# alessandroragano/nomad

Hardware: AMD Instinct MI355X
Metric: clips/sec embedded + NxM NOMAD distances, 16kHz x 4s batches (higher is better)
Workload: dtype f32; 1 GPU; configs[1]: batch=256 x 64000 samples (T=199) per GPU, wav2vec2-base + projection head fp32, 224 deg x 32*N ref float64 distances + means; deg_per_gpu=224, ref_total=32, parallelism=clip-sharded x1, all-gather of ref embeddings, collective=none (single process, no process group)

## Files before the change

### nomad_amd/build.py

```python
from __future__ import annotations

import os
import shutil
import subprocess
import time

HERE = os.path.dirname(os.path.abspath(__file__))
CSRC = os.path.join(HERE, "csrc")
LIB = os.path.join(HERE, "libnomad_hip.so")
DIAG_LIB = os.path.join(HERE, "libnomad_diag.so")
SOURCES = ["nomad_hip.hip", "nomad_gemm_f32.hip", "nomad_gemm_bf16.hip"]
HEADERS = sorted(f for f in os.listdir(CSRC) if f.endswith(".h")) + [os.path.join("..", "..", "include", "nomad_hip.h")]


def hipcc_path() -> str:
    for cand in (os.environ.get("HIPCC"), shutil.which("hipcc"), "/opt/rocm/bin/hipcc"):
        if cand and os.path.exists(cand):
            return cand
    raise RuntimeError("hipcc not found; the HIP libraries cannot be built")


def needs_build(lib: str = LIB) -> bool:
    if not os.path.exists(lib):
        return True
    t = os.path.getmtime(lib)
    deps = [os.path.join(CSRC, s) for s in SOURCES + HEADERS] + [os.path.abspath(__file__)]
    return any(os.path.getmtime(d) > t for d in deps if os.path.exists(d))


NO_PACKED_FP32 = ["-Xclang", "-target-feature", "-Xclang", "-packed-fp32-ops"]


def pk_path(lib: str) -> str:
    return lib[:-3] + "_pk.so"


VARIANTS = {"gelu1": ["-DNOMAD_GELU_BF16_FORM=1"],
            "gelu2": ["-DNOMAD_GELU_BF16_FORM=2"],
            "poswino1": ["-DNOMAD_POSCONV_WINO_LEVELS=1"],
            "gelu_tail6": ["-DNOMAD_GELU_F32_FORM=2"]}


def variant_path(lib: str, name: str) -> str:
    return lib[:-3] + f"_{name}.so"


def _flags(lib: str, diag: bool, verbose: bool):
    flags = ["--offload-arch=gfx950", "-O3", "-std=c++17", "-fPIC", "-Wall", "-Wno-unused-function", "-pthread"]
    for name, defs in VARIANTS.items():
        if lib.endswith(f"_{name}.so"):
            flags = defs + flags
    if os.environ.get("NOMAD_PACKED_FP32", "0") != "1" and not lib.endswith("_pk.so"):
        flags = NO_PACKED_FP32 + flags
    else:
        flags.insert(0, "-DNOMAD_PACKED_FP32_BUILD=1")
    if diag:
        flags.insert(0, "-DNOMAD_DIAG")
    if verbose:
        flags.insert(0, "-Rpass-analysis=kernel-resource-usage")
    return flags


class _Job:

    def __init__(self, lib: str, diag: bool, verbose: bool = False):
        self.lib, self.t0 = lib, time.perf_counter()
        self.tmp = lib + f".tmp{os.getpid()}"
        self.flags = _flags(lib, diag, verbose)
        self.objs = [f"{lib}.{os.path.splitext(s)[0]}.{os.getpid()}.o" for s in SOURCES]
        self.procs = [subprocess.Popen([hipcc_path(), *self.flags, "-c", os.path.join(CSRC, s), "-o", o],
                                       stdout=subprocess.PIPE, stderr=subprocess.PIPE, text=True) for s, o in zip(SOURCES, self.objs)]

    def _cleanup(self):
        for f in self.objs + [self.tmp]:
            if os.path.exists(f):
                os.remove(f)

    def finish(self) -> float:
        errs = []
        for p in self.procs:
            out, err = p.communicate()
            if p.returncode != 0:
                errs.append(out + err)
        if errs:
            self._cleanup()
            raise RuntimeError("hipcc failed:\n" + "\n".join(errs))
        link = subprocess.run([hipcc_path(), "--offload-arch=gfx950", "-shared", "-fPIC", "-pthread", "-o", self.tmp, *self.objs],
                              capture_output=True, text=True)
        if link.returncode != 0:
            self._cleanup()
            raise RuntimeError("hipcc (link) failed:\n" + link.stdout + link.stderr)
        os.replace(self.tmp, self.lib)
        self._cleanup()
# ... 37 lines not shown
```

### nomad_amd/csrc/conv_s2_f32.hip.h

```cpp
#pragma once
#include "gemm_f32.hip.h"

namespace nomad {

struct ConvS2Params {
    const float* X;
    const float* W;
    float* Y;
    float* Upre;
    int pairs;
    int tiles_m;
    int L, Lin, ppc;
    unsigned ppc_magic;
    int ppc_shift;
    const int* pp;
    const int* opref;
    const int* ipref;
    int nclips;
};

struct ConvS2Cfg {
    static constexpr int BMP = 128, BN = 128, NT = 512;
    static constexpr int STAGE = 8 * 1024 + 132;
    static constexpr int ZOFF = 8 * 1024;
    static constexpr int LDS_BYTES = 2 * STAGE * 4;
};

struct PairRows {
    long long in0, in_last, out0;
    bool odd_ok;
};

template <bool RAGGED>
__device__ __forceinline__ PairRows conv_s2_pair(const ConvS2Params& p, int s) {
    PairRows r;
    if (RAGGED) {
        int lo = 0, hi = p.nclips;
        while (hi - lo > 1) {
            const int mid = (lo + hi) >> 1;
            if (p.pp[mid] <= s) lo = mid;
            else hi = mid;
        }
        const int j = s - p.pp[lo];
        const int L = p.opref[lo + 1] - p.opref[lo];
        r.in0 = (long long)p.ipref[lo] + 4 * j;
        r.in_last = (long long)p.ipref[lo + 1] - 1;
        r.out0 = (long long)p.opref[lo] + 2 * j;
        r.odd_ok = 2 * j + 1 < L;
    } else {
        const int c = p.ppc_magic ? fast_div(s, p.ppc_magic, p.ppc_shift) : (p.ppc == 1 ? s : 0);
        const int j = s - c * p.ppc;
        r.in0 = (long long)c * p.Lin + 4 * j;
        r.in_last = (long long)c * p.Lin + p.Lin - 1;
        r.out0 = (long long)c * p.L + 2 * j;
        r.odd_ok = 2 * j + 1 < p.L;
    }
    return r;
}

template <bool RAGGED>
__global__ __launch_bounds__(512, 4) void conv_s2_f32_kernel(const ConvS2Params p) {
    using Cfg = ConvS2Cfg;
    extern __shared__ __attribute__((aligned(16))) float smem[];
    const int tid = threadIdx.x, lane = tid & 63;
    const int wave = __builtin_amdgcn_readfirstlane(tid >> 6);
    const int wm = wave >> 1, wn = wave & 1;
    const int nwg = p.tiles_m * 4;
    const int wg = xcd_remap(blockIdx.x, nwg);
    const int tile_m = wg >> 2, tile_n = wg & 3;
    const int m0 = tile_m * Cfg::BMP, n0 = tile_n * Cfg::BN;

    if (tid < 2 * 33) *reinterpret_cast<f32x4*>(smem + (tid / 33) * Cfg::STAGE + Cfg::ZOFF + (tid % 33) * 4) = (f32x4){0.f, 0.f, 0.f, 0.f};

    const long long tile_in0 = conv_s2_pair<RAGGED>(p, m0).in0;
    const float* const a_tile = uniform_ptr(p.X + tile_in0 * 512);
    const float* const b_tile = uniform_ptr(p.W + (long long)n0 * 1536);
    int v1a, v1b;
    {
        const int r1 = tid >> 2, lc = (tid & 3) ^ ((r1 >> 2) & 3);
        const int s = min(m0 + r1, p.pairs - 1);
        const PairRows pr = conv_s2_pair<RAGGED>(p, s);
        v1a = (int)(((pr.in0 + 2 - tile_in0) * 512 + lc * 4) * 4);
        v1b = (r1 * 1536 + lc * 4) * 4;
    }
    const int f0 = wave >> 2;
    int v2a[3], v2b;
    {
        const int r = (tid & 255) >> 1, lc = (tid & 1) ^ ((r >> 3) & 1);
        const int s = min(m0 + r, p.pairs - 1);
        const PairRows pr = conv_s2_pair<RAGGED>(p, s);
#pragma unroll
        for (int i = 0; i < 3; ++i) {
            const int f = i == 2 ? 4 : f0 + 2 * i;
            const long long row = min(pr.in0 + f, pr.in_last);
            v2a[i] = (int)(((row - tile_in0) * 512 + lc * 4) * 4);
        }
        v2b = (r * 1536 + lc * 4) * 4;
    }
    auto issue = [&](const int q, const int buf) {
        float* st = smem + buf * Cfg::STAGE + wave * 256;
        if (q < 32) {
            const int k0 = q * 16;
            dma16_buffer(a_tile, (lptr_t)(st), v1a, k0 * 4);
            dma16_buffer(b_tile, (lptr_t)(st + 2048), v1b, k0 * 4);
            dma16_buffer(b_tile, (lptr_t)(st + 4096), v1b, (k0 + 1024) * 4);
        } else {
            const int k0 = (q - 32) * 8;
            dma16_buffer(a_tile, (lptr_t)(st), v2a[0], k0 * 4);
            dma16_buffer(a_tile, (lptr_t)(st + 2048), v2a[1], k0 * 4);
            if (f0 == 0) dma16_buffer(a_tile, (lptr_t)(st + 4096), v2a[2], k0 * 4);
            else dma16_buffer(b_tile, (lptr_t)(st + 4096), v2b, k0 * 4);
            dma16_buffer(b_tile, (lptr_t)(st + 6144), v2b, ((1 + f0) * 512 + k0) * 4);
        }
    };

    const int fi = lane & 15, g = lane >> 4;
    const int ra = wm * 32 + fi, rb = wn * 64 + fi;
    const int sw1 = (g ^ ((fi >> 2) & 3)) * 4;
    const int o1a = ra * 16 + sw1, o1b = 2048 + rb * 16 + sw1;
    const int sw2 = ((g & 1) ^ (fi >> 3)) * 4;
    const bool lo = g < 2;
    const int oEF = (lo ? 0 : 1024) + ra * 8 + sw2;
    const int oES = lo ? 2048 + ra * 8 + sw2 : Cfg::ZOFF;
    const int oOF = (lo ? 3072 : 4096) + ra * 8 + sw2;
    const int oOS = lo ? Cfg::ZOFF : 2048 + ra * 8 + sw2;
    const int oBE = (lo ? 5120 : 6144) + rb * 8 + sw2;
    const int oBO = (lo ? 6144 : 7168) + rb * 8 + sw2;

    f32x4 E[2][4], O[2][4];
#pragma unroll
    for (int si = 0; si < 2; ++si)
#pragma unroll
        for (int sj = 0; sj < 4; ++sj) E[si][sj] = (f32x4){0.f, 0.f, 0.f, 0.f};

    auto rd = [&](const float* base, int off) { return *reinterpret_cast<const f32x4*>(base + off); };
    auto mm = [&](f32x4 (&acc)[2][4], const f32x4 (&a)[2], const f32x4 (&b)[4]) {
#pragma unroll
        for (int c = 0; c < 4; ++c)
#pragma unroll
            for (int si = 0; si < 2; ++si)
#pragma unroll
                for (int sj = 0; sj < 4; ++sj) acc[si][sj] = __builtin_amdgcn_mfma_f32_16x16x4f32(b[sj][c], a[si][c], acc[si][sj], 0, 0, 0);
    };
    auto step1 = [&](const float* st) {
        f32x4 a[2], b[4];
#pragma unroll
        for (int si = 0; si < 2; ++si) a[si] = rd(st, o1a + si * 256);
#pragma unroll
        for (int sj = 0; sj < 4; ++sj) {
            const f32x4 u = rd(st, o1b + sj * 256), v = rd(st, o1b + 2048 + sj * 256);
#pragma unroll
            for (int e = 0; e < 4; ++e) b[sj][e] = u[e] + v[e];
        }
        mm(E, a, b);
    };
    auto operand = [&](const float* st, int of, int os, f32x4 (&a)[2]) {
#pragma unroll
        for (int si = 0; si < 2; ++si) {
            const f32x4 u = rd(st, of + si * 128), v = rd(st, os + si * 128);
#pragma unroll
            for (int e = 0; e < 4; ++e) a[si][e] = u[e] - v[e];
        }
    };
    auto step2 = [&](const float* st) {
        f32x4 a[2], b[4];
        operand(st, oEF, oES, a);
#pragma unroll
        for (int sj = 0; sj < 4; ++sj) b[sj] = rd(st, oBE + sj * 128);
        mm(E, a, b);
        asm volatile("" ::: "memory");
        __builtin_amdgcn_sched_barrier(0);
        operand(st, oOF, oOS, a);
#pragma unroll
        for (int sj = 0; sj < 4; ++sj) b[sj] = rd(st, oBO + sj * 128);
        mm(O, a, b);
    };

    auto wait_step = [] {
        asm volatile("s_waitcnt vmcnt(0)" ::: "memory");
        __syncthreads();
    };
    float* const st0 = smem;
    float* const st1 = smem + Cfg::STAGE;
    issue(0, 0);
    for (int q = 0; q < 32; q += 2) {
        wait_step();
        issue(q + 1, 1);
        step1(st0);
        wait_step();
        issue(q + 2, 0);
        step1(st1);
    }
#pragma unroll
    for (int si = 0; si < 2; ++si)
#pragma unroll
        for (int sj = 0; sj < 4; ++sj) O[si][sj] = E[si][sj];
    for (int q = 32; q < 96; q += 2) {
        wait_step();
        issue(q + 1, 1);
        step2(st0);
        wait_step();
        if (q + 2 < 96) issue(q + 2, 0);
        step2(st1);
    }

    int lane_e = lane;
    asm volatile("" : "+v"(lane_e));
    const int col = n0 + wn * 64 + 4 * (lane_e >> 4);
#pragma unroll
    for (int si = 0; si < 2; ++si) {
        const int s = m0 + wm * 32 + (lane_e & 15) + 16 * si;
        if (s >= p.pairs) continue;
        const PairRows pr = conv_s2_pair<RAGGED>(p, s);
        const long long ie = pr.out0 * 512 + col, io = ie + 512;
#pragma unroll
        for (int sj = 0; sj < 4; ++sj) {
            f32x4 ve = E[si][sj], vo = O[si][sj];
            if (p.Upre) {
                *reinterpret_cast<f32x4*>(p.Upre + ie + sj * 16) = ve;
                if (pr.odd_ok) *reinterpret_cast<f32x4*>(p.Upre + io + sj * 16) = vo;
            }
#pragma unroll
            for (int e = 0; e < 4; ++e) {
                ve[e] = gelu_erf(ve[e]);
                vo[e] = gelu_erf(vo[e]);
            }
            *reinterpret_cast<f32x4*>(p.Y + ie + sj * 16) = ve;
            if (pr.odd_ok) *reinterpret_cast<f32x4*>(p.Y + io + sj * 16) = vo;
        }
    }
}

}
```

### nomad_amd/csrc/nomad_ctx.hip.h

```cpp
#pragma once
#include <hip/hip_runtime.h>

#include <algorithm>
#include <cmath>
#include <cstdarg>
#include <cstdio>
#include <cstdlib>
#include <cstring>
#include <atomic>
#include <mutex>
#include <string>
#include <vector>

#include "../../include/nomad_hip.h"

#include "dtypes.hip.h"
#include "gemm_f32.hip.h"

#define NOMAD_INTERNAL __attribute__((visibility("hidden")))

using namespace nomad;

inline thread_local char g_err[512] = "";

// ... 20 lines not shown
constexpr long long kPairScratchDoubles = 1 << 21;
constexpr int kCdistMaxD = 4096;
constexpr int kEventChunk = 8192;
const int* const kNoInts = nullptr;
const hipStream_t kNoStream = reinterpret_cast<hipStream_t>(~uintptr_t(0));

}

struct LayerDev {
    float *qkv_w, *qkv_b, *o_w, *o_b, *ln1_w, *ln1_b, *fc1_w, *fc1_b, *fc2_w, *fc2_b, *ln2_w, *ln2_b;
};


struct Tuning {
    bool splitk_lnb_fuse = true;
    bool splitk_ln_fuse = true;
    bool f32_conv_wino = true;
    bool f32_posconv_wino = true;
    int bf16_attn_tail = 0;
    int bf16_ln_rows = 4;
    int p9_short = 1;
    bool attn_bwd_small = true;
    bool p9_wl = false;
    bool p9_late = true;
    int p9_skew = 0;
    int concurrent_parts = 1;
};

#ifdef NOMAD_DIAG
static void tuning_from_env(Tuning& t) {
    auto geti = [](const char* n, int d) { const char* e = getenv(n); return e ? atoi(e) : d; };
    auto getb = [](const char* n, bool d) { const char* e = getenv(n); return e ? atoi(e) != 0 : d; };
    t.splitk_ln_fuse = getb("NOMAD_SPLITK_LN", t.splitk_ln_fuse);
    t.splitk_lnb_fuse = getb("NOMAD_SPLITK_LNB", t.splitk_lnb_fuse);
    t.f32_conv_wino = getb("NOMAD_F32_CONV_WINO", t.f32_conv_wino);
    t.f32_posconv_wino = getb("NOMAD_F32_POSCONV_WINO", t.f32_posconv_wino);
    t.bf16_attn_tail = geti("NOMAD_BF16_ATTN_TAIL", t.bf16_attn_tail);
    t.bf16_ln_rows = geti("NOMAD_BF16_LN_ROWS", t.bf16_ln_rows);
    t.p9_short = geti("NOMAD_BF16_P9_SHORT", t.p9_short);
    t.p9_skew = geti("NOMAD_BF16_P9_SKEW", t.p9_skew);
    t.p9_late = getb("NOMAD_BF16_P9_LATE", t.p9_late);
    t.p9_wl = getb("NOMAD_BF16_P9_WL", t.p9_wl);
    t.attn_bwd_small = getb("NOMAD_ATTN_BWD_SMALL", t.attn_bwd_small);
}
#endif

struct nomad_ctx {
    int device = 0;
    int num_cus = 256;
    Tuning tune;
    bool keep = false;
    float* conv0_w = nullptr;
    float* conv_w[7] = {};
    float *gn_w = nullptr, *gn_b = nullptr, *fln_w = nullptr, *fln_b = nullptr;
    float *proj_w = nullptr, *proj_b = nullptr;
    float *pos_w = nullptr, *pos_b = nullptr;
    float* pos_wt = nullptr;
    float *eln_w = nullptr, *eln_b = nullptr;
    LayerDev layers[NOMAD_NUM_LAYERS] = {};
    float *emb_w = nullptr, *emb_b = nullptr;
    float* splitk_part = nullptr;
    float* splitk_cur = nullptr;
    size_t splitk_cur_floats = 0;
    bool splitk_ok = false;
    struct PendingLn {
        const float* gamma = nullptr;
        const float* beta = nullptr;
        float* out = nullptr;
        float* out2 = nullptr;
        bool armed = false, done = false;
    } pending_ln;
    struct PendingLnBwd {
        const float* x = nullptr;
        const float* g2 = nullptr;
        const float* gamma = nullptr;
        float* out = nullptr;
        bool armed = false, done = false;
    } pending_lnb;
    std::vector<std::pair<hipStream_t, double*>> pair_scratch;
    std::mutex pair_mu;
    bool bwd_ready = false;
    float* conv_bw_even[7] = {};
    float* conv_bw_odd[7] = {};
    float* conv_bw2[7] = {};
    float* proj_wT = nullptr;
    float* pos_wb = nullptr;
    float *qkv_wT[NOMAD_NUM_LAYERS] = {}, *o_wT[NOMAD_NUM_LAYERS] = {}, *fc1_wT[NOMAD_NUM_LAYERS] = {},
          *fc2_wT[NOMAD_NUM_LAYERS] = {};
    bool bf16_ready = false;
    bf16_t* conv_w16[7] = {};
    bf16_t* conv0_wfrag = nullptr;
    bf16_t *proj_w16 = nullptr, *pos_w16 = nullptr;
    bf16_t* pos_wfrag16 = nullptr;
    bf16_t *qkv_w16[NOMAD_NUM_LAYERS] = {}, *o_w16[NOMAD_NUM_LAYERS] = {}, *fc1_w16[NOMAD_NUM_LAYERS] = {},
           *fc2_w16[NOMAD_NUM_LAYERS] = {};
    float* qkv_b16[NOMAD_NUM_LAYERS] = {};
    bool x3_ready = false;
    bf16s_t* conv_wx[7] = {};
    bf16s_t* proj_wx = nullptr;
    bf16s_t* pos_wx = nullptr;
    float* pos_bx = nullptr;
    bf16s_t *qkv_wx[NOMAD_NUM_LAYERS] = {}, *o_wx[NOMAD_NUM_LAYERS] = {}, *fc1_wx[NOMAD_NUM_LAYERS] = {},
            *fc2_wx[NOMAD_NUM_LAYERS] = {};
    bool train_ready = false;
    float *theta = nullptr, *grad = nullptr, *adam_m = nullptr, *adam_v = nullptr;
    double *pos_nrm2 = nullptr, *tap_partial = nullptr, *tap_dot = nullptr;
// ... 53 lines not shown
        c->p_fl[cls] += flops;
        c->p_n[cls] += 1;
        if (cls2 >= 0) {
            c->p_fl[cls2] += flops;
            c->p_n[cls2] += 1;
        }
        slot = c->ev_used;
        c->ev_class[slot / 2] = cls | ((cls2 + 1) << 8);
        c->ev_used += 2;
        (void)hipEventRecord(c->ev[slot], s);
    }
    ~Scope() {
        if (slot >= 0) (void)hipEventRecord(c->ev[slot + 1], s);
    }
};

RowMap plain_map(int M, int ld) { return RowMap{0, 0, M > 0 ? M : 1, ld}; }

int occ_pad(int occ, int lds) {
    if (occ <= 0) return 0;
    const int budget = (160 * 1024 / occ) & ~255;
    return budget > lds ? budget - lds : 0;
}

GemmParams dense(const float* A, int lda, const float* W, const float* bias, const float* R, float* C, int M, int N,
                 int K, int gelu) {
    GemmParams p{};
    p.A = A;
    p.amap = plain_map(M, lda);
    p.kchunk = K;
    p.kstride = 0;
    p.W = W;
    p.ldw = K;
    p.C = C;
    p.cmap = plain_map(M, N);
    p.bias = bias;
    p.R = R;
    p.rmap = plain_map(M, N);
    p.M = M;
    p.N = N;
    p.K = K;
    p.n_valid = N;
    p.gelu = gelu;
    return p;
}

}

NOMAD_INTERNAL int run_gemm(nomad_ctx* c, GemmParams p, int groups, int tile, hipStream_t s, int occ = 0);
NOMAD_INTERNAL int gemm_f32_dispatch(nomad_ctx* c, GemmParams p, int groups, int tile, hipStream_t s, int occ);
NOMAD_INTERNAL hipError_t gemm_f32_n48_split(const GemmParams& q, int groups, hipStream_t s, int S);
NOMAD_INTERNAL int pick_tile(const nomad_ctx* c, int M, int N, int K);
NOMAD_INTERNAL int mixed_split_rows(const nomad_ctx* c, int M, int N);
NOMAD_INTERNAL int run_conv_s2_f32(nomad_ctx* c, const float* X, const float* W, float* Y, float* Upre, int B, int Lin, int L,
                                   const int* pp, const int* opref, const int* ipref, int pairs, hipStream_t s);
NOMAD_INTERNAL int run_gemm_bf16(nomad_ctx* c, GemmParams p, int groups, hipStream_t s, int tile = -1);
#ifdef NOMAD_DIAG
NOMAD_INTERNAL int gemm_f32_timeline_read(unsigned long long* out_host, int n);
NOMAD_INTERNAL int gemm_bf16_timeline_read(unsigned long long* out_host, int n);
#endif
```

### nomad_amd/csrc/nomad_gemm_f32.hip

```cpp
#include "nomad_ctx.hip.h"
#include "conv_s2_f32.hip.h"

int gemm_f32_dispatch(nomad_ctx* c, GemmParams p, int groups, int tile, hipStream_t s, int occ) {
    if (tile == 29 && occ == 0) occ = 4;
    const double flops = 2.0 * p.M * (double)p.n_valid * p.K * groups;
    Scope sc(c, s, NOMAD_K_GEMM, flops, tile == 33 ? NOMAD_K_GEMM_BIG : ((tile == 34 || tile == 31 || tile == 48) ? NOMAD_K_GEMM_FINE : -1));
    hipError_t e;
    if (c->gemm_x3 && tile == 48 && p.N == 64)
        tile = 37;
    if (c->gemm_x3 && (tile == 31 || tile == 34 || tile == 37) && p.N % 128 == 0 &&
        (long long)((p.M + 127) / 128) * (p.N / 128) >= 512)
        tile = 20;
    const bool plain_cr = p.c_colblk == 0 && p.cmap.clip_rows >= p.M && !p.cmap.pref &&
                          (!p.R || (p.rmap.clip_rows >= p.M && !p.rmap.pref)) && (!p.DG || (p.dgmap.clip_rows >= p.M && !p.dgmap.pref));
    if (c->gemm_x3 && plain_cr && (tile == 20 || tile == 31 || tile == 34 || tile == 37)) {
        constexpr int T = 16 | 32;
        switch (tile) {
            case 20: e = launch_gemm_glds<128, 128, 32, 2, 2, 2, false, 12 | T, true>(p, groups, s, occ_pad(occ, GldsCfg<128, 128, 32, 2, 2>::LDS_BYTES)); break;
            case 31: e = launch_gemm_glds<128, 128, 32, 4, 2, 2, false, 12 | T, true>(p, groups, s, occ_pad(occ, GldsCfg<128, 128, 32, 4, 2>::LDS_BYTES)); break;
            case 34: e = launch_gemm_glds<128, 64, 32, 4, 2, 3, false, 12 | T, true>(p, groups, s); break;
            default: e = launch_gemm_glds<64, 64, 32, 2, 2, 3, false, 12 | T, true>(p, groups, s); break;
        }
        if (e != hipSuccess) return fail(NOMAD_ERR_HIP, "gemm (bf16x3 products) launch: %s", hipGetErrorString(e));
        return 0;
// ... 212 lines not shown
        Scope sc(c, st, NOMAD_K_GEMM, 2.0 * M * (double)N * K, NOMAD_K_GEMM_BIG);
        constexpr int V = 13 | 16 | 64 | 16384;
        if (R) HIP_TRY((launch_gemm_mixed<V | 32768, V | 32768>(pp, m1, st)));
        else HIP_TRY((launch_gemm_mixed<V | 1024, V | 1024>(pp, m1, st)));
        return 0;
    }
    if (tile == 97 || tile == 98) {
        if (N % 128 || K % 32 || gelu || !R) return fail(NOMAD_ERR_INVALID, "nomad_diag_gemm: tile %d needs N %% 128 == 0, K %% 32 == 0, a residual and no GELU", tile);
        GemmParams pp = dense(A, K, W, bias, R, C, M, N, K, gelu);
        hipStream_t st = static_cast<hipStream_t>(stream);
        Scope sc(c, st, NOMAD_K_GEMM, 2.0 * M * (double)N * K, NOMAD_K_GEMM_BIG);
        if (tile == 97) HIP_TRY((launch_gemm_glds<256, 128, 16, 4, 2, 3, false, 13 | 16 | 64 | 16384 | 32768>(pp, 1, st)));
        else HIP_TRY((launch_gemm_glds<128, 128, 32, 4, 2, 2, false, 12 | 16 | 16384 | 32768>(pp, 1, st, occ_pad(0, GldsCfg<128, 128, 32, 4, 2>::LDS_BYTES))));
        return 0;
    }
    if (tile >= 88 && tile <= 93) {
        if (N % 128 || K % 32) return fail(NOMAD_ERR_INVALID, "nomad_diag_gemm: N %% 128 or K %% 32 != 0");
        GemmParams pp = dense(A, K, W, bias, R, C, M, N, K, gelu);
        hipStream_t st = static_cast<hipStream_t>(stream);
        Scope sc(c, st, NOMAD_K_GEMM, 2.0 * M * (double)N * K, NOMAD_K_GEMM_BIG);
        constexpr int L = 16384;
        switch (tile) {
            case 88: HIP_TRY((launch_gemm_glds<256, 128, 16, 4, 2, 3, false, 13 | 16 | L>(pp, 1, st))); break;
            case 89: HIP_TRY((launch_gemm_glds<256, 128, 16, 4, 2, 3, false, 13 | 16 | 1024 | L>(pp, 1, st))); break;
            case 90: HIP_TRY((launch_gemm_glds<256, 128, 16, 4, 2, 3, false, 13 | 16 | 64 | 1024 | L>(pp, 1, st))); break;
            case 91: HIP_TRY((launch_gemm_glds<256, 128, 16, 4, 2, 3, false, 13 | 16 | 64 | L>(pp, 1, st))); break;
            case 92: HIP_TRY((launch_gemm_glds<128, 128, 32, 4, 2, 2, false, 12 | 16 | L>(pp, 1, st, occ_pad(0, GldsCfg<128, 128, 32, 4, 2>::LDS_BYTES)))); break;
            default: HIP_TRY((launch_gemm_glds<128, 128, 32, 4, 2, 2, false, 12 | 16 | 1024 | L>(pp, 1, st, occ_pad(0, GldsCfg<128, 128, 32, 4, 2>::LDS_BYTES)))); break;
        }
        return 0;
    }
    if (tile == 84 || tile == 85) {
        if (N % 128 || K % 16) return fail(NOMAD_ERR_INVALID, "nomad_diag_gemm: N %% 128 or K %% 16 != 0");
        GemmParams pp = dense(A, K, W, bias, R, C, M, N, K, gelu);
        Scope sc(c, static_cast<hipStream_t>(stream), NOMAD_K_GEMM, 2.0 * M * (double)N * K, NOMAD_K_GEMM_BIG);
        if (tile == 85) return fail(NOMAD_ERR_INVALID, "nomad_diag_gemm: tile 85 (BK = 8) went with the 16x16x4 products (16-deep k groups)");
        HIP_TRY((launch_gemm_glds<256, 128, 16, 4, 2, 3, false, 13 | 16 | 64 | 1024>(pp, 1, static_cast<hipStream_t>(stream))));
        return 0;
    }
#else
    if (tile == 84 || tile == 85 || (tile >= 88 && tile <= 95) || (tile >= 97 && tile <= 99))
        return fail(NOMAD_ERR_INVALID, "gemm tile id %d is not in this library (experimental instantiations live in libnomad_diag.so)", tile);
#endif
    if (tile < 0 || (tile > 47 && (tile < 60 || tile > 81) && tile != 86)) return fail(NOMAD_ERR_INVALID, "nomad_diag_gemm: tile id %d", tile);
    const int bn = (tile == 46 || tile == 47) ? 64 : tile >= 60 ? (tile == 67 ? 256 : 128) : kBN[tile], bk = tile == 46 ? 32 : tile == 47 ? 16 : tile >= 60 ? (tile == 73 ? 32 : 16) : kBK[tile];
    if (N % bn || K % bk) return fail(NOMAD_ERR_INVALID, "nomad_diag_gemm: N %% %d or K %% %d != 0", bn, bk);
    GemmParams p = dense(A, K, W, bias, R, C, M, N, K, gelu);
    p.group_m = group_m;
    return run_gemm(c, p, 1, tile, static_cast<hipStream_t>(stream), occ);
}

}

int run_conv_s2_f32(nomad_ctx* c, const float* X, const float* W, float* Y, float* Upre, int B, int Lin, int L, const int* pp,
                    const int* opref, const int* ipref, int pairs, hipStream_t s) {
    ConvS2Params p{};
    p.X = X;
    p.W = W;
    p.Y = Y;
    p.Upre = Upre;
    p.pairs = pairs;
    p.tiles_m = (pairs + ConvS2Cfg::BMP - 1) / ConvS2Cfg::BMP;
    p.nclips = B;
    if (ipref) {
        p.pp = pp;
        p.opref = opref;
        p.ipref = ipref;
    } else {
        p.L = L;
        p.Lin = Lin;
        p.ppc = (L + 1) / 2;
        if (Lin < 2 * L + 1 || pairs != B * p.ppc) return fail(NOMAD_ERR_INVALID, "conv_s2: %d clips of %d -> %d frames, %d pairs", B, Lin, L, pairs);
        p.ppc_magic = 0;
        p.ppc_shift = 0;
        if (B > 1 && p.ppc > 1) fast_div_magic((unsigned)p.ppc, &p.ppc_magic, &p.ppc_shift);
    }
    const double flops = 2.0 * (double)pairs * 512 * 2560;
    Scope sc(c, s, NOMAD_K_GEMM, flops, NOMAD_K_GEMM_BIG);
    static LdsAttrOnce attr_u, attr_r;
    hipError_t e;
    if (ipref) {
        if ((e = attr_r.ensure(reinterpret_cast<const void*>(conv_s2_f32_kernel<true>), ConvS2Cfg::LDS_BYTES)) != hipSuccess)
            return fail(NOMAD_ERR_HIP, "conv_s2 attribute: %s", hipGetErrorString(e));
        hipLaunchKernelGGL(conv_s2_f32_kernel<true>, dim3(p.tiles_m * 4), dim3(ConvS2Cfg::NT), ConvS2Cfg::LDS_BYTES, s, p);
    } else {
        if ((e = attr_u.ensure(reinterpret_cast<const void*>(conv_s2_f32_kernel<false>), ConvS2Cfg::LDS_BYTES)) != hipSuccess)
            return fail(NOMAD_ERR_HIP, "conv_s2 attribute: %s", hipGetErrorString(e));
        hipLaunchKernelGGL(conv_s2_f32_kernel<false>, dim3(p.tiles_m * 4), dim3(ConvS2Cfg::NT), ConvS2Cfg::LDS_BYTES, s, p);
    }
    if ((e = hipGetLastError()) != hipSuccess) return fail(NOMAD_ERR_HIP, "conv_s2 launch: %s", hipGetErrorString(e));
    return 0;
}

#ifdef NOMAD_DIAG
extern "C" {
int nomad_diag_conv_s2(nomad_ctx* c, const float* X, const float* W, float* Y, float* U, int B, const int* lin_host, int ragged,
                       void* stream) {
    if (!c || !X || !W || !Y || !lin_host || B <= 0) return fail(NOMAD_ERR_INVALID, "nomad_diag_conv_s2: bad argument");
    std::vector<int> meta(3 * (size_t)(B + 1), 0);
    for (int b = 0; b < B; ++b) {
        const int lin = lin_host[b], L = lin >= 3 ? (lin - 3) / 2 + 1 : 0;
        if (L <= 0 || (!ragged && lin != lin_host[0])) return fail(NOMAD_ERR_INVALID, "nomad_diag_conv_s2: clip %d of %d frames", b, lin);
        meta[b + 1] = meta[b] + (L + 1) / 2;
        meta[(B + 1) + b + 1] = meta[(B + 1) + b] + L;
        meta[2 * (B + 1) + b + 1] = meta[2 * (B + 1) + b] + lin;
    }
    hipStream_t s = static_cast<hipStream_t>(stream);
    int* d = nullptr;
    HIP_TRY(hipMalloc(&d, sizeof(int) * meta.size()));
    int rc = 0;
    if (hipMemcpy(d, meta.data(), sizeof(int) * meta.size(), hipMemcpyHostToDevice) != hipSuccess) rc = fail(NOMAD_ERR_HIP, "nomad_diag_conv_s2: copy");
    const int lin0 = lin_host[0], L0 = (lin0 - 3) / 2 + 1;
    if (rc == 0)
        rc = ragged ? run_conv_s2_f32(c, X, W, Y, U, B, 0, 0, d, d + (B + 1), d + 2 * (B + 1), meta[B], s)
                    : run_conv_s2_f32(c, X, W, Y, U, B, lin0, L0, nullptr, nullptr, nullptr, meta[B], s);
    if (rc == 0 && hipStreamSynchronize(s) != hipSuccess) rc = fail(NOMAD_ERR_HIP, "nomad_diag_conv_s2: kernel");
    (void)hipFree(d);
    return rc;
}
}
#endif
```

### nomad_amd/csrc/nomad_hip.hip

```cpp
#include "nomad_ctx.hip.h"

#include "attention.hip.h"
#include "attention_bf16_v3.hip.h"
#include "posconv_bf16_slab.hip.h"
#include "attention_f32_v2.hip.h"
#include "attention_bwd.hip.h"
#include "backward.hip.h"
#include "frontend.hip.h"
#include "gemm_bf16.hip.h"
#include "gemm_bf16_8phase.hip.h"
#include "gemm_bf16_p9.hip.h"
#include "gemm_bf16x3.hip.h"
#include "gemm_f32.hip.h"
#ifdef NOMAD_DIAG
#endif
#include "pairwise.hip.h"
#include "posconv_wino_f32.hip.h"
#include "rowops.hip.h"
#include "train.hip.h"
#include "wav_reader.h"

namespace {

struct Shapes {
// ... 763 lines not shown
            if ((long long)m.size() < info[i].frames) m.resize((size_t)info[i].frames);
            status[i] = wav::read_one(paths[i], info[i], m.data(), raw[(size_t)t]);
            if (status[i] != NOMAD_OK) return;
            if (kern_rate[(size_t)t] != info[i].sample_rate) {
                kern[(size_t)t] = wav::make_resample_kernel(info[i].sample_rate, target_rate);
                kern_rate[(size_t)t] = info[i].sample_rate;
            }
            wav::resample_into(m.data(), info[i].frames, kern[(size_t)t], dst,
                               wav::resampled_frames(info[i].frames, info[i].sample_rate, target_rate));
        });
    } catch (const std::exception& e) {
        return fail(NOMAD_ERR_IO, "nomad_wav_read_rows: %s", e.what());
    }
    for (int i = 0; i < n; ++i)
        if (status[i] != NOMAD_OK) return fail(status[i], "nomad_wav_read_rows: %s: %s", paths[i], status[i] == NOMAD_ERR_IO ? "read failed" : "unsupported encoding");
    return NOMAD_OK;
}

int nomad_num_frames(int n_samples) {
    Shapes s;
    return make_shapes(1, n_samples, &s) ? s.T : 0;
}

int nomad_create(nomad_ctx** out, int device, const nomad_weights* w) {
    if (!out || !w) return fail(NOMAD_ERR_INVALID, "nomad_create: null argument");
    int ndev = 0;
    if (hipGetDeviceCount(&ndev) != hipSuccess || ndev <= 0 || device < 0 || device >= ndev)
        return fail(NOMAD_ERR_NO_DEVICE, "nomad_create: no HIP device %d (count %d); this engine has no CPU path",
                    device, ndev);
    hipDeviceProp_t prop;
    HIP_TRY(hipGetDeviceProperties(&prop, device));
    if (strncmp(prop.gcnArchName, "gfx950", 6) != 0)
        return fail(NOMAD_ERR_NO_DEVICE, "nomad_create: device %d is %s, kernels are built for gfx950 only", device,
                    prop.gcnArchName);
    HIP_TRY(hipSetDevice(device));
    nomad_ctx* c = new nomad_ctx();
    c->device = device;
    c->num_cus = prop.multiProcessorCount > 0 ? prop.multiProcessorCount : 256;
#ifdef NOMAD_DIAG
    tuning_from_env(c->tune);
#endif
    int rc = 0;
    auto up = [&](const float* h, size_t n, float** d) {
        if (rc == 0) rc = upload(c, h, n, d);
    };
    up(w->conv_w[0], 512 * 10, &c->conv0_w);
    for (int i = 1; i < 7 && rc == 0; ++i) {
        const int k = kConvK[i];
        std::vector<float> r((size_t)512 * k * 512);
        for (int n = 0; n < 512; ++n)
            for (int ci = 0; ci < 512; ++ci)
                for (int t = 0; t < k; ++t) r[(size_t)n * k * 512 + t * 512 + ci] = w->conv_w[i][((size_t)n * 512 + ci) * k + t];
        up(r.data(), r.size(), &c->conv_w[i]);
    }
    up(w->gn_w, 512, &c->gn_w);
    up(w->gn_b, 512, &c->gn_b);
    up(w->feat_ln_w, 512, &c->fln_w);
    up(w->feat_ln_b, 512, &c->fln_b);
    up(w->proj_w, 768 * 512, &c->proj_w);
    up(w->proj_b, 768, &c->proj_b);
    if (rc == 0) {
        std::vector<double> nrm(128, 0.0);
        for (size_t o = 0; o < 768; ++o)
            for (size_t ci = 0; ci < 48; ++ci)
                for (size_t t = 0; t < 128; ++t) {
                    const double v = w->pos_v[(o * 48 + ci) * 128 + t];
                    nrm[t] += v * v;
                }
        std::vector<float> sc(128);
        for (int t = 0; t < 128; ++t) sc[t] = (float)((double)w->pos_g[t] / std::sqrt(nrm[t]));
        std::vector<float> r((size_t)16 * 64 * 6144, 0.f);
        for (size_t g = 0; g < 16; ++g)
            for (size_t n = 0; n < 48; ++n)
                for (size_t ci = 0; ci < 48; ++ci)
                    for (size_t t = 0; t < 128; ++t)
                        r[(g * 64 + n) * 6144 + t * 48 + ci] = w->pos_v[((g * 48 + n) * 48 + ci) * 128 + t] * sc[t];
        up(r.data(), r.size(), &c->pos_w);
        if (rc == 0 && c->tune.f32_posconv_wino) {
            void* d = nullptr;
            const hipError_t e = hipMalloc(&d, sizeof(float) * 16 * kPwOps * 64 * kPwK);
            if (e != hipSuccess) rc = fail(NOMAD_ERR_HIP, "nomad_create: pos-conv weights: %s", hipGetErrorString(e));
            else {
                c->allocs.push_back(d);
                c->pos_wt = static_cast<float*>(d);
                rc = rebuild_posconv_wino_weights(c, nullptr);
                if (rc == 0 && hipStreamSynchronize(nullptr) != hipSuccess) rc = fail(NOMAD_ERR_HIP, "nomad_create: pos-conv weights: kernel");
            }
        }
    }
    up(w->pos_b, 768, &c->pos_b);
    up(w->enc_ln_w, 768, &c->eln_w);
    up(w->enc_ln_b, 768, &c->eln_b);
    for (int l = 0; l < NOMAD_NUM_LAYERS && rc == 0; ++l) {
        const nomad_layer_weights& lw = w->layers[l];
        LayerDev& d = c->layers[l];
        std::vector<float> qkv((size_t)2304 * 768), qb(2304);
        for (size_t i = 0; i < (size_t)768 * 768; ++i) {
            qkv[i] = lw.q_w[i] * 0.125f;
            qkv[(size_t)768 * 768 + i] = lw.k_w[i];
            qkv[(size_t)2 * 768 * 768 + i] = lw.v_w[i];
        }
        for (int i = 0; i < 768; ++i) {
            qb[i] = lw.q_b[i] * 0.125f;
            qb[768 + i] = lw.k_b[i];
            qb[1536 + i] = lw.v_b[i];
        }
// ... 84 lines not shown
    float *pwq = nullptr, *pws = nullptr;
    int* pwmeta = nullptr;
};

static int forward_run(nomad_ctx* c, const float* wav, const BatchGeom& g, const F32Bufs& bf, const float* head_w,
                       const float* head_b, float* emb, float* layers_out, float* splitk_block, size_t splitk_floats, hipStream_t s,
                       const Saved* sv, bool features = false) {
    if (g.ragged() && splitk_block) return fail(NOMAD_ERR_INVALID, "fp32 forward: split-K needs an equal-length batch");
    const int B = g.B, T = g.T, M = (int)g.rows[6];
    const int depth = c->encoder_depth;
    if (depth < NOMAD_NUM_LAYERS && (!layers_out || features)) return refuse_cut(c, "fp32 forward");
    float* const loss_block = (sv == nullptr && layers_out != nullptr && splitk_block != nullptr) ? splitk_block : nullptr;
    const SplitKScope splitk(c, (sv != nullptr || loss_block != nullptr) && !c->train_ready && !g.ragged());
    float* const prev_cur = c->splitk_cur;
    const size_t prev_cur_floats = c->splitk_cur_floats;
    c->splitk_cur = sv != nullptr ? c->splitk_part : loss_block;
    c->splitk_cur_floats = sv != nullptr ? kSplitKPartFloats : loss_block != nullptr ? splitk_floats : 0;
    struct CurRestore {
        nomad_ctx* c;
        float* v;
        size_t n;
        ~CurRestore() { c->splitk_cur = v; c->splitk_cur_floats = n; }
    } cur_restore{c, prev_cur, prev_cur_floats};
    int rc;
    const bool reg = sv != nullptr;
    const DropCfg d_in = make_drop(c, reg ? c->p_input : 0.f), d_res = make_drop(c, reg ? c->p_drop : 0.f),
                  d_att = make_drop(c, reg ? c->p_attn : 0.f);
    int nbr = 1;
    unsigned bmask[4] = {reg ? c->layer_mask : 0xFFFu, 0xFFFu, 0xFFFu, 0xFFFu};
    if (reg && c->branches > 1) {
        if (B % c->branches) return fail(NOMAD_ERR_INVALID, "nomad_embed_train: B=%d is not %d equal branches", B, c->branches);
        nbr = c->branches;
        for (int i = 0; i < nbr; ++i) bmask[i] = c->branch_mask[i];
    }
    const long long act = (long long)M * 768;

    float* gn_scale = sv ? sv->gn_scale : bf.scale;
    float* gn_shift = sv ? sv->gn_shift : bf.shift;
    {
        Scope sc(c, s, NOMAD_K_FRONT, 0.0);
        launch_wav_stats(wav, g.wav_ld, g.L[0], g.max_l0, B, bf.stats, g.lens, s);
        hipLaunchKernelGGL(gn_fold_kernel, dim3(B), dim3(512), 0, s, bf.stats, c->conv0_w, c->gn_w, c->gn_b, g.L[0],
                           gn_scale, gn_shift, sv ? sv->gn_mean : nullptr, sv ? sv->gn_rstd : nullptr, g.lens);
    }
    {
        Scope sc(c, s, NOMAD_K_FRONT, 2.0 * (double)g.rows[0] * 512 * 10);
        hipLaunchKernelGGL(conv0_gn_gelu_kernel<float>, dim3((g.max_l0 + kConv0Frames - 1) / kConv0Frames, B), dim3(256), 0, s,
                           wav, g.wav_ld, g.L[0], c->conv0_w, gn_scale, gn_shift, bf.conv[0], g.lens, g.pref[0]);
    }
    HIP_TRY(hipGetLastError());

    for (int i = 1; i < 7; ++i) {
        if (conv_wino(c, i)) {
            if ((rc = run_conv_s2_f32(c, bf.conv[i - 1], c->conv_w[i], bf.conv[i], sv ? sv->u[i] : nullptr, B, g.L[i - 1], g.L[i],
                                      g.pairpref[i], g.pref[i], g.pref[i - 1], (int)g.pairs[i], s)))
                return rc;
            continue;
        }
        GemmParams p{};
        p.A = bf.conv[i - 1];
        p.amap = g.conv_amap[i];
        p.K = kConvK[i] * 512;
        p.kchunk = p.K;
        p.W = c->conv_w[i];
        p.ldw = p.K;
        p.C = (sv && i == 6) ? sv->c6 : bf.conv[i];
        p.Upre = sv ? sv->u[i] : nullptr;
        p.M = (int)g.rows[i];
        p.N = 512;
        p.n_valid = 512;
        p.cmap = plain_map(p.M, 512);
        p.rmap = p.cmap;
        p.gelu = 1;
        if ((rc = run_gemm(c, p, 1, pick_tile(c, p.M, 512, p.K), s))) return rc;
    }

    if ((rc = run_layernorm(c, sv ? sv->c6 : bf.conv[6], c->fln_w, c->fln_b, bf.featln, nullptr, M, 512, s)))
        return rc;
    float* xpad = bf.xpad;
    {
        Scope sc(c, s, NOMAD_K_ROW, 0.0);
        hipLaunchKernelGGL(zero_pad_rows_kernel<float>, dim3(16 * B), dim3(256), 0, s, xpad, T, g.pref[6], g.ppref, B);
    }
    {
        GemmParams p = dense(bf.featln, 512, c->proj_w, c->proj_b, nullptr, xpad, M, 768, 512, 0);
        p.cmap = g.pad_map;
        p.c_colblk = 48;
        p.c_colblk_stride = g.grp_stride;
        if ((rc = run_gemm(c, p, 1, pick_tile(c, M, 768, 512), s))) return rc;
    }
    if (d_in.threshold) {
        Scope sc(c, s, NOMAD_K_ROW, 0.0);
        hipLaunchKernelGGL(dropout_groups_kernel, dim3(M), dim3(192), 0, s, xpad, T, g.grp_stride, d_in, kSiteInput, g.pref[6], g.ppref, B);
    }
    if (posconv_wino(c)) {
        if (!bf.pwq || !bf.pws) return fail(NOMAD_ERR_INVALID, "fp32 forward: no workspace for the pos-conv operands");
        if ((rc = run_posconv_wino(c, xpad, c->pos_wt, c->pos_b, sv ? sv->y0 : bf.y, sv ? sv->upc : nullptr, g.pos_wino, bf.pwq, bf.pws, bf.pwmeta, s)))
            return rc;
    } else {
        GemmParams p{};
        p.A = xpad;
        p.amap = g.pos_amap;
        p.a_goff = g.grp_stride;
        p.K = 6144;
        p.kchunk = 6144;
        p.W = c->pos_w;
        p.ldw = 6144;
        p.w_goff = 64LL * 6144;
// ... 1707 lines not shown
            v.push_back({b + "self_attn.out_proj.bias", q.o_b, 768});
            v.push_back({b + "self_attn_layer_norm.weight", q.ln1_w, 768});
            v.push_back({b + "self_attn_layer_norm.bias", q.ln1_b, 768});
            v.push_back({b + "fc1.weight", q.fc1_w, (size_t)3072 * 768});
            v.push_back({b + "fc1.bias", q.fc1_b, 3072});
            v.push_back({b + "fc2.weight", q.fc2_w, (size_t)768 * 3072});
            v.push_back({b + "fc2.bias", q.fc2_b, 768});
            v.push_back({b + "final_layer_norm.weight", q.ln2_w, 768});
            v.push_back({b + "final_layer_norm.bias", q.ln2_b, 768});
        }
        const std::string fe = p + "feature_extractor.conv_layers.";
        v.push_back({fe + "0.0.weight", o.conv0_w, 512 * 10});
        v.push_back({fe + "0.2.weight", o.gn_w, 512});
        v.push_back({fe + "0.2.bias", o.gn_b, 512});
        for (int i = 1; i < 7; ++i) v.push_back({fe + std::to_string(i) + ".0.weight", o.conv_w[i], (size_t)512 * 512 * kConvK[i]});
        v.push_back({"embedding_layer.1.weight", o.emb_w, 256 * 768});
        v.push_back({"embedding_layer.1.bias", o.emb_b, 256});
        return v;
    }();
    return segs;
}

void rebuild_conv_bwd_weights(nomad_ctx* c, hipStream_t s) {
    auto transpose = [&](const float* in, int ld_in, float* out, int ld_out, int R, int C) {
        hipLaunchKernelGGL(transpose_kernel, dim3((C + 31) / 32, (R + 31) / 32), dim3(32, 8), 0, s, in, ld_in, out, ld_out, R, C);
    };
    for (int i = 1; i <= 4; ++i) {
        transpose(c->conv_w[i] + 2 * 512, 1536, c->conv_bw_even[i], 1024, 512, 512);
        transpose(c->conv_w[i], 1536, c->conv_bw_even[i] + 512, 1024, 512, 512);
        transpose(c->conv_w[i] + 512, 1536, c->conv_bw_odd[i], 512, 512, 512);
    }
    for (int i = 5; i <= 6; ++i)
        transpose(c->conv_w[i], 1024, c->conv_bw2[i], 512, 512, 1024);
}

int refresh_weights(nomad_ctx* c, hipStream_t s) {
    const ParamOffsets po = make_param_offsets();
    auto transpose = [&](const float* in, int ld_in, float* out, int ld_out, int R, int C) {
        hipLaunchKernelGGL(transpose_kernel, dim3((C + 31) / 32, (R + 31) / 32), dim3(32, 8), 0, s, in, ld_in, out, ld_out, R, C);
    };
    hipLaunchKernelGGL(tap_dot_partial_kernel, dim3(576), dim3(256), 0, s, c->theta + po.pos_v, (const float*)nullptr,
                       c->tap_partial);
    hipLaunchKernelGGL(tap_sum_final_kernel, dim3(1), dim3(1024), 0, s, c->tap_partial, 576, c->pos_nrm2);
    hipLaunchKernelGGL(posconv_fold_kernel, dim3(768), dim3(256), 0, s, c->theta + po.pos_v, c->theta + po.pos_g,
                       c->pos_nrm2, c->pos_w);
    hipLaunchKernelGGL(posconv_bwd_weight_kernel, dim3(16 * 64), dim3(256), 0, s, c->pos_w, c->pos_wb);
    if (c->pos_wt)
        if (int rc = rebuild_posconv_wino_weights(c, s)) return rc;
    transpose(c->proj_w, 512, c->proj_wT, 768, 768, 512);
    for (int i = 1; i < 7; ++i) {
        const long long n = 512LL * 512 * kConvK[i];
        hipLaunchKernelGGL(conv_repack_kernel, dim3((unsigned)((n + 255) / 256)), dim3(256), 0, s, c->theta + po.conv_w[i], c->conv_w[i],
                           kConvK[i]);
    }
    rebuild_conv_bwd_weights(c, s);
    for (int l = 0; l < NOMAD_NUM_LAYERS; ++l) {
        const LayerDev& d = c->layers[l];
        const LayerOffsets& lo = po.L[l];
        const long long w4 = (long long)2304 * 768 / 4, q4 = (long long)768 * 768 / 4;
        hipLaunchKernelGGL(scale_rows_kernel, dim3((unsigned)((w4 + 255) / 256)), dim3(256), 0, s,
                           reinterpret_cast<const float4*>(c->theta + lo.qkv_w), reinterpret_cast<float4*>(d.qkv_w), w4, q4, 0.125f);
        hipLaunchKernelGGL(scale_rows_kernel, dim3(3), dim3(256), 0, s, reinterpret_cast<const float4*>(c->theta + lo.qkv_b),
                           reinterpret_cast<float4*>(d.qkv_b), 576LL, 192LL, 0.125f);
        transpose(d.qkv_w, 768, c->qkv_wT[l], 2304, 2304, 768);
        transpose(d.o_w, 768, c->o_wT[l], 768, 768, 768);
        transpose(d.fc1_w, 768, c->fc1_wT[l], 3072, 3072, 768);
        transpose(d.fc2_w, 3072, c->fc2_wT[l], 768, 768, 3072);
    }
    HIP_TRY(hipGetLastError());
    c->bf16_ready = false;
    c->x3_ready = false;
    return 0;
}

}

extern "C" {

int nomad_set_gemm_precision(nomad_ctx* c, int mode) {
    if (!c || (mode != 0 && mode != 1)) return fail(NOMAD_ERR_INVALID, "nomad_set_gemm_precision: mode must be 0 (fp32 MFMA) or 1 (bf16x3 products)");
    c->gemm_x3 = mode;
    return 0;
}

int nomad_get_gemm_precision(const nomad_ctx* c, int* mode) {
    if (!c || !mode) return fail(NOMAD_ERR_INVALID, "nomad_get_gemm_precision: null argument");
    *mode = c->gemm_x3;
    return 0;
}

int nomad_set_feature_grad_mult(nomad_ctx* c, float mult) {
    if (!c || !(mult >= 0.f)) return fail(NOMAD_ERR_INVALID, "nomad_set_feature_grad_mult: bad argument");
    c->feature_grad_mult = mult;
    return 0;
}

int nomad_get_feature_grad_mult(const nomad_ctx* c, float* mult) {
    if (!c || !mult) return fail(NOMAD_ERR_INVALID, "nomad_get_feature_grad_mult: bad argument");
    *mult = c->feature_grad_mult;
    return 0;
}

int nomad_set_encoder_depth(nomad_ctx* c, int depth) {
    if (!c || depth < 1 || depth > NOMAD_NUM_LAYERS)
        return fail(NOMAD_ERR_INVALID, "nomad_set_encoder_depth: depth %d is outside 1 .. %d", depth, NOMAD_NUM_LAYERS);
    c->encoder_depth = depth;
// ... 632 lines not shown
```

Before: 2492 clips/s.

## Precompute conv tap-sum weight plane and widen phase-1 stages to 32 channels

The stride-2 Winograd-style conv kernel used to load two weight taps and add them in registers during phase 1. That sum is now precomputed once into a separate weight plane, which is rebuilt whenever the weights are refreshed, so phase 1 loads one weight tile and does no per-step adds. By default the phase-1 stage is also widened to 32 input channels per step, which halves the number of phase-1 pipeline iterations and swaps in a new LDS swizzle. Other lever combinations are exposed as build variants. The cost is an extra 1 MB buffer per layer, plus a risk of LDS bank conflicts with the new 32-wide swizzle.

```diff
diff --git a/nomad_amd/build.py b/nomad_amd/build.py
--- a/nomad_amd/build.py
+++ b/nomad_amd/build.py
@@ -38,7 +38,9 @@
 VARIANTS = {"gelu1": ["-DNOMAD_GELU_BF16_FORM=1"],
             "gelu2": ["-DNOMAD_GELU_BF16_FORM=2"],
             "poswino1": ["-DNOMAD_POSCONV_WINO_LEVELS=1"],
-            "gelu_tail6": ["-DNOMAD_GELU_F32_FORM=2"]}
+            "gelu_tail6": ["-DNOMAD_GELU_F32_FORM=2"],
+            "cs2_r7": ["-DNOMAD_CONV_S2_LEVERS=0"], "cs2_plane": ["-DNOMAD_CONV_S2_LEVERS=1"], "cs2_all": ["-DNOMAD_CONV_S2_LEVERS=7"],
+            "cs2_clean": ["-DNOMAD_CONV_S2_LEVERS=4"]}
 
 
 def variant_path(lib: str, name: str) -> str:
diff --git a/nomad_amd/csrc/conv_s2_f32.hip.h b/nomad_amd/csrc/conv_s2_f32.hip.h
--- a/nomad_amd/csrc/conv_s2_f32.hip.h
+++ b/nomad_amd/csrc/conv_s2_f32.hip.h
@@ -6,6 +6,7 @@
 struct ConvS2Params {
     const float* X;
     const float* W;
+    const float* S;
     float* Y;
     float* Upre;
     int pairs;
@@ -19,12 +20,32 @@
     int nclips;
 };
 
+#ifndef NOMAD_CONV_S2_LEVERS
+#define NOMAD_CONV_S2_LEVERS 3
+#endif
+
 struct ConvS2Cfg {
+    static constexpr bool PLANE = NOMAD_CONV_S2_LEVERS & 1, K32 = NOMAD_CONV_S2_LEVERS & 2, CLEAN = NOMAD_CONV_S2_LEVERS & 4;
+    static_assert(PLANE || !K32, "a 32-channel phase-1 stage is f2 + the tap-sum plane");
+    static constexpr int P1 = K32 ? 16 : 32, NQ = P1 + 64;
+    static __host__ __device__ constexpr int swz8(int r) { return CLEAN ? 0 : (r >> 3) & 1; }
+    static __host__ __device__ constexpr int swz16(int r) { return CLEAN ? (r >> 2) & 2 : (r >> 2) & 3; }
+    static __host__ __device__ constexpr int swz32(int r) { return (r >> 1) & 7; }
     static constexpr int BMP = 128, BN = 128, NT = 512;
     static constexpr int STAGE = 8 * 1024 + 132;
     static constexpr int ZOFF = 8 * 1024;
     static constexpr int LDS_BYTES = 2 * STAGE * 4;
 };
+
+__global__ __launch_bounds__(256) void conv_s2_plane_kernel(const float* __restrict__ W, float* __restrict__ S) {
+    const int i = blockIdx.x * 256 + threadIdx.x, n = i >> 7, c = (i & 127) * 4;
+    const f32x4 u = *reinterpret_cast<const f32x4*>(W + (long long)n * 1536 + c);
+    const f32x4 v = *reinterpret_cast<const f32x4*>(W + (long long)n * 1536 + 1024 + c);
+    f32x4 r;
+#pragma unroll
+    for (int e = 0; e < 4; ++e) r[e] = u[e] + v[e];
+    *reinterpret_cast<f32x4*>(S + (long long)n * 512 + c) = r;
+}
 
 struct PairRows {
     long long in0, in_last, out0;
@@ -75,18 +96,23 @@
     const long long tile_in0 = conv_s2_pair<RAGGED>(p, m0).in0;
     const float* const a_tile = uniform_ptr(p.X + tile_in0 * 512);
     const float* const b_tile = uniform_ptr(p.W + (long long)n0 * 1536);
-    int v1a, v1b;
+    const float* const s_tile = uniform_ptr((Cfg::PLANE ? p.S : p.W) + (long long)n0 * 512);
+    int v1a[2], v1b;
     {
-        const int r1 = tid >> 2, lc = (tid & 3) ^ ((r1 >> 2) & 3);
-        const int s = min(m0 + r1, p.pairs - 1);
-        const PairRows pr = conv_s2_pair<RAGGED>(p, s);
-        v1a = (int)(((pr.in0 + 2 - tile_in0) * 512 + lc * 4) * 4);
-        v1b = (r1 * 1536 + lc * 4) * 4;
+        const int r1 = Cfg::K32 ? tid >> 3 : tid >> 2;
+        const int lc = Cfg::K32 ? (tid & 7) ^ Cfg::swz32(r1) : (tid & 3) ^ Cfg::swz16(r1);
+#pragma unroll
+        for (int i = 0; i < 2; ++i) {
+            const int s = min(m0 + r1 + 64 * i, p.pairs - 1);
+            const PairRows pr = conv_s2_pair<RAGGED>(p, s);
+            v1a[i] = (int)(((pr.in0 + 2 - tile_in0) * 512 + lc * 4) * 4);
+        }
+        v1b = (r1 * (Cfg::PLANE ? 512 : 1536) + lc * 4) * 4;
     }
     const int f0 = wave >> 2;
     int v2a[3], v2b;
     {
-        const int r = (tid & 255) >> 1, lc = (tid & 1) ^ ((r >> 3) & 1);
+        const int r = (tid & 255) >> 1, lc = (tid & 1) ^ Cfg::swz8(r);
         const int s = min(m0 + r, p.pairs - 1);
         const PairRows pr = conv_s2_pair<RAGGED>(p, s);
 #pragma unroll
@@ -99,13 +125,25 @@
     }
     auto issue = [&](const int q, const int buf) {
         float* st = smem + buf * Cfg::STAGE + wave * 256;
-        if (q < 32) {
-            const int k0 = q * 16;
-            dma16_buffer(a_tile, (lptr_t)(st), v1a, k0 * 4);
-            dma16_buffer(b_tile, (lptr_t)(st + 2048), v1b, k0 * 4);
-            dma16_buffer(b_tile, (lptr_t)(st + 4096), v1b, (k0 + 1024) * 4);
+        if (q < Cfg::P1) {
+            if (Cfg::K32) {
+                const int k0 = q * 32;
+                dma16_buffer(a_tile, (lptr_t)(st), v1a[0], k0 * 4);
+                dma16_buffer(a_tile, (lptr_t)(st + 2048), v1a[1], k0 * 4);
+                dma16_buffer(s_tile, (lptr_t)(st + 4096), v1b, k0 * 4);
+                dma16_buffer(s_tile, (lptr_t)(st + 6144), v1b, (64 * 512 + k0) * 4);
+            } else if (Cfg::PLANE) {
+                const int k0 = q * 16;
+                dma16_buffer(a_tile, (lptr_t)(st), v1a[0], k0 * 4);
+                dma16_buffer(s_tile, (lptr_t)(st + 2048), v1b, k0 * 4);
+            } else {
+                const int k0 = q * 16;
+                dma16_buffer(a_tile, (lptr_t)(st), v1a[0], k0 * 4);
+                dma16_buffer(b_tile, (lptr_t)(st + 2048), v1b, k0 * 4);
+                dma16_buffer(b_tile, (lptr_t)(st + 4096), v1b, (k0 + 1024) * 4);
+            }
         } else {
-            const int k0 = (q - 32) * 8;
+            const int k0 = (q - Cfg::P1) * 8;
             dma16_buffer(a_tile, (lptr_t)(st), v2a[0], k0 * 4);
             dma16_buffer(a_tile, (lptr_t)(st + 2048), v2a[1], k0 * 4);
             if (f0 == 0) dma16_buffer(a_tile, (lptr_t)(st + 4096), v2a[2], k0 * 4);
@@ -116,9 +154,9 @@
 
     const int fi = lane & 15, g = lane >> 4;
     const int ra = wm * 32 + fi, rb = wn * 64 + fi;
-    const int sw1 = (g ^ ((fi >> 2) & 3)) * 4;
-    const int o1a = ra * 16 + sw1, o1b = 2048 + rb * 16 + sw1;
-    const int sw2 = ((g & 1) ^ (fi >> 3)) * 4;
+    const int sw1 = Cfg::K32 ? (g ^ Cfg::swz32(fi)) * 4 : (g ^ Cfg::swz16(fi)) * 4;
+    const int o1a = ra * (Cfg::K32 ? 32 : 16) + sw1, o1b = (Cfg::K32 ? 4096 + rb * 32 : 2048 + rb * 16) + sw1;
+    const int sw2 = ((g & 1) ^ Cfg::swz8(fi)) * 4;
     const bool lo = g < 2;
     const int oEF = (lo ? 0 : 1024) + ra * 8 + sw2;
     const int oES = lo ? 2048 + ra * 8 + sw2 : Cfg::ZOFF;
@@ -144,10 +182,26 @@
     };
     auto step1 = [&](const float* st) {
         f32x4 a[2], b[4];
+        if (Cfg::K32) {
+#pragma unroll
+            for (int h = 0; h < 2; ++h) {
+                const int oa = h ? o1a ^ 16 : o1a, ob = h ? o1b ^ 16 : o1b;
+#pragma unroll
+                for (int si = 0; si < 2; ++si) a[si] = rd(st, oa + si * 512);
+#pragma unroll
+                for (int sj = 0; sj < 4; ++sj) b[sj] = rd(st, ob + sj * 512);
+                mm(E, a, b);
+            }
+            return;
+        }
 #pragma unroll
         for (int si = 0; si < 2; ++si) a[si] = rd(st, o1a + si * 256);
 #pragma unroll
         for (int sj = 0; sj < 4; ++sj) {
+            if (Cfg::PLANE) {
+                b[sj] = rd(st, o1b + sj * 256);
+                continue;
+            }
             const f32x4 u = rd(st, o1b + sj * 256), v = rd(st, o1b + 2048 + sj * 256);
 #pragma unroll
             for (int e = 0; e < 4; ++e) b[sj][e] = u[e] + v[e];
@@ -183,7 +237,7 @@
     float* const st0 = smem;
     float* const st1 = smem + Cfg::STAGE;
     issue(0, 0);
-    for (int q = 0; q < 32; q += 2) {
+    for (int q = 0; q < Cfg::P1; q += 2) {
         wait_step();
         issue(q + 1, 1);
         step1(st0);
@@ -195,12 +249,12 @@
     for (int si = 0; si < 2; ++si)
 #pragma unroll
         for (int sj = 0; sj < 4; ++sj) O[si][sj] = E[si][sj];
-    for (int q = 32; q < 96; q += 2) {
+    for (int q = Cfg::P1; q < Cfg::NQ; q += 2) {
         wait_step();
         issue(q + 1, 1);
         step2(st0);
         wait_step();
-        if (q + 2 < 96) issue(q + 2, 0);
+        if (q + 2 < Cfg::NQ) issue(q + 2, 0);
         step2(st1);
     }
 
diff --git a/nomad_amd/csrc/nomad_ctx.hip.h b/nomad_amd/csrc/nomad_ctx.hip.h
--- a/nomad_amd/csrc/nomad_ctx.hip.h
+++ b/nomad_amd/csrc/nomad_ctx.hip.h
@@ -96,6 +96,7 @@
     bool keep = false;
     float* conv0_w = nullptr;
     float* conv_w[7] = {};
+    float* conv_s[7] = {};
     float *gn_w = nullptr, *gn_b = nullptr, *fln_w = nullptr, *fln_b = nullptr;
     float *proj_w = nullptr, *proj_b = nullptr;
     float *pos_w = nullptr, *pos_b = nullptr;
@@ -255,8 +256,9 @@
 NOMAD_INTERNAL hipError_t gemm_f32_n48_split(const GemmParams& q, int groups, hipStream_t s, int S);
 NOMAD_INTERNAL int pick_tile(const nomad_ctx* c, int M, int N, int K);
 NOMAD_INTERNAL int mixed_split_rows(const nomad_ctx* c, int M, int N);
-NOMAD_INTERNAL int run_conv_s2_f32(nomad_ctx* c, const float* X, const float* W, float* Y, float* Upre, int B, int Lin, int L,
-                                   const int* pp, const int* opref, const int* ipref, int pairs, hipStream_t s);
+NOMAD_INTERNAL int run_conv_s2_f32(nomad_ctx* c, const float* X, const float* W, const float* S, float* Y, float* Upre, int B, int Lin,
+                                   int L, const int* pp, const int* opref, const int* ipref, int pairs, hipStream_t s);
+NOMAD_INTERNAL int rebuild_conv_s2_plane(const float* W, float* S, hipStream_t s);
 NOMAD_INTERNAL int run_gemm_bf16(nomad_ctx* c, GemmParams p, int groups, hipStream_t s, int tile = -1);
 #ifdef NOMAD_DIAG
 NOMAD_INTERNAL int gemm_f32_timeline_read(unsigned long long* out_host, int n);
diff --git a/nomad_amd/csrc/nomad_gemm_f32.hip b/nomad_amd/csrc/nomad_gemm_f32.hip
--- a/nomad_amd/csrc/nomad_gemm_f32.hip
+++ b/nomad_amd/csrc/nomad_gemm_f32.hip
@@ -288,11 +288,19 @@
 
 }
 
-int run_conv_s2_f32(nomad_ctx* c, const float* X, const float* W, float* Y, float* Upre, int B, int Lin, int L, const int* pp,
-                    const int* opref, const int* ipref, int pairs, hipStream_t s) {
+int rebuild_conv_s2_plane(const float* W, float* S, hipStream_t s) {
+    hipLaunchKernelGGL(conv_s2_plane_kernel, dim3(512 * 128 / 256), dim3(256), 0, s, W, S);
+    HIP_TRY(hipGetLastError());
+    return 0;
+}
+
+int run_conv_s2_f32(nomad_ctx* c, const float* X, const float* W, const float* S, float* Y, float* Upre, int B, int Lin, int L,
+                    const int* pp, const int* opref, const int* ipref, int pairs, hipStream_t s) {
+    if (!S) return fail(NOMAD_ERR_INVALID, "conv_s2: no tap-sum plane");
     ConvS2Params p{};
     p.X = X;
     p.W = W;
+    p.S = S;
     p.Y = Y;
     p.Upre = Upre;
     p.pairs = pairs;
@@ -344,15 +352,28 @@
     hipStream_t s = static_cast<hipStream_t>(stream);
     int* d = nullptr;
     HIP_TRY(hipMalloc(&d, sizeof(int) * meta.size()));
+    float* plane = nullptr;
+    if (hipMalloc(&plane, sizeof(float) * 512 * 512) != hipSuccess) {
+        (void)hipFree(d);
+        return fail(NOMAD_ERR_HIP, "nomad_diag_conv_s2: plane");
+    }
     int rc = 0;
     if (hipMemcpy(d, meta.data(), sizeof(int) * meta.size(), hipMemcpyHostToDevice) != hipSuccess) rc = fail(NOMAD_ERR_HIP, "nomad_diag_conv_s2: copy");
     const int lin0 = lin_host[0], L0 = (lin0 - 3) / 2 + 1;
+    if (rc == 0) rc = rebuild_conv_s2_plane(W, plane, s);
     if (rc == 0)
-        rc = ragged ? run_conv_s2_f32(c, X, W, Y, U, B, 0, 0, d, d + (B + 1), d + 2 * (B + 1), meta[B], s)
-                    : run_conv_s2_f32(c, X, W, Y, U, B, lin0, L0, nullptr, nullptr, nullptr, meta[B], s);
-    if (rc == 0 && hipStreamSynchronize(s) != hipSuccess) rc = fail(NOMAD_ERR_HIP, "nomad_diag_conv_s2: kernel");
+        rc = ragged ? run_conv_s2_f32(c, X, W, plane, Y, U, B, 0, 0, d, d + (B + 1), d + 2 * (B + 1), meta[B], s)
+                    : run_conv_s2_f32(c, X, W, plane, Y, U, B, lin0, L0, nullptr, nullptr, nullptr, meta[B], s);
+    if (hipStreamSynchronize(s) != hipSuccess && rc == 0) rc = fail(NOMAD_ERR_HIP, "nomad_diag_conv_s2: kernel");
+    (void)hipFree(plane);
     (void)hipFree(d);
     return rc;
 }
+
+int nomad_diag_conv_s2_plane(nomad_ctx* c, int layer, float* dst) {
+    if (!c || !dst || layer < 1 || layer > 4 || !c->conv_s[layer]) return fail(NOMAD_ERR_INVALID, "nomad_diag_conv_s2_plane: bad argument");
+    HIP_TRY(hipMemcpy(dst, c->conv_s[layer], sizeof(float) * 512 * 512, hipMemcpyDeviceToDevice));
+    return 0;
+}
 }
 #endif
diff --git a/nomad_amd/csrc/nomad_hip.hip b/nomad_amd/csrc/nomad_hip.hip
--- a/nomad_amd/csrc/nomad_hip.hip
+++ b/nomad_amd/csrc/nomad_hip.hip
@@ -839,6 +839,17 @@
             for (int ci = 0; ci < 512; ++ci)
                 for (int t = 0; t < k; ++t) r[(size_t)n * k * 512 + t * 512 + ci] = w->conv_w[i][((size_t)n * 512 + ci) * k + t];
         up(r.data(), r.size(), &c->conv_w[i]);
+        if (rc == 0 && kConvK[i] == 3) {
+            void* d = nullptr;
+            const hipError_t e = hipMalloc(&d, sizeof(float) * 512 * 512);
+            if (e != hipSuccess) rc = fail(NOMAD_ERR_HIP, "nomad_create: conv tap-sum plane: %s", hipGetErrorString(e));
+            else {
+                c->allocs.push_back(d);
+                c->conv_s[i] = static_cast<float*>(d);
+                rc = rebuild_conv_s2_plane(c->conv_w[i], c->conv_s[i], nullptr);
+                if (rc == 0 && hipStreamSynchronize(nullptr) != hipSuccess) rc = fail(NOMAD_ERR_HIP, "nomad_create: conv tap-sum plane: kernel");
+            }
+        }
     }
     up(w->gn_w, 512, &c->gn_w);
     up(w->gn_b, 512, &c->gn_b);
@@ -1029,8 +1040,8 @@
 
     for (int i = 1; i < 7; ++i) {
         if (conv_wino(c, i)) {
-            if ((rc = run_conv_s2_f32(c, bf.conv[i - 1], c->conv_w[i], bf.conv[i], sv ? sv->u[i] : nullptr, B, g.L[i - 1], g.L[i],
-                                      g.pairpref[i], g.pref[i], g.pref[i - 1], (int)g.pairs[i], s)))
+            if ((rc = run_conv_s2_f32(c, bf.conv[i - 1], c->conv_w[i], c->conv_s[i], bf.conv[i], sv ? sv->u[i] : nullptr, B, g.L[i - 1],
+                                      g.L[i], g.pairpref[i], g.pref[i], g.pref[i - 1], (int)g.pairs[i], s)))
                 return rc;
             continue;
         }
@@ -2844,6 +2855,8 @@
         const long long n = 512LL * 512 * kConvK[i];
         hipLaunchKernelGGL(conv_repack_kernel, dim3((unsigned)((n + 255) / 256)), dim3(256), 0, s, c->theta + po.conv_w[i], c->conv_w[i],
                            kConvK[i]);
+        if (c->conv_s[i])
+            if (int rc = rebuild_conv_s2_plane(c->conv_w[i], c->conv_s[i], s)) return rc;
     }
     rebuild_conv_bwd_weights(c, s);
     for (int l = 0; l < NOMAD_NUM_LAYERS; ++l) {
```

Result: no change. 2509 clips/s (median of 6 runs) (+0.7%).
